# andrewmagis/snap-rnaseq

Measured on AMD Instinct MI355X. Metric: aligned reads/sec (100 bp SE, k=20 seed) at 1/2/4/8 GPUs + CPU baseline, higher is better.
Workload: dtype u8

## Files before the change

include/snapgpu.h:

```cpp
#ifndef SNAPGPU_H
#define SNAPGPU_H

#include <stddef.h>
#include <stdint.h>

#ifdef __cplusplus
extern "C" {
#endif

#define SNAPGPU_ABI_VERSION 2

enum {
    SNAPGPU_OK = 0,
    SNAPGPU_EINVAL = -1,
    SNAPGPU_EIO = -2,
    SNAPGPU_ENOMEM = -3,
    SNAPGPU_EDEVICE = -4,
    SNAPGPU_EFORMAT = -5,
    SNAPGPU_EUNSUPPORTED = -6
};

enum { SNAPGPU_NOT_FOUND = 0, SNAPGPU_SINGLE_HIT = 1, SNAPGPU_MULTIPLE_HITS = 2, SNAPGPU_UNKNOWN = 3 };
enum { SNAPGPU_FORWARD = 0, SNAPGPU_RC = 1 };

// ... 170 lines not shown
    uint32_t location;
    uint8_t  direction;
    uint8_t  score;
    uint16_t reserved;
} snapgpu_multi_hit_t;
int snapgpu_align_batch_ex(snapgpu_aligner_t *a, const snapgpu_reads_t *reads, const snapgpu_search_t *search,
                           uint32_t maxHitsToGet, snapgpu_result_t *out, int32_t *multiHitsFound,
                           snapgpu_multi_hit_t *multiHits);

typedef struct snapgpu_device_reads snapgpu_device_reads_t;
snapgpu_device_reads_t *snapgpu_reads_upload(snapgpu_aligner_t *a, const snapgpu_reads_t *reads);
void snapgpu_device_reads_free(snapgpu_device_reads_t *d);
int  snapgpu_align_resident(snapgpu_aligner_t *a, snapgpu_device_reads_t *d);
int  snapgpu_results_download(snapgpu_aligner_t *a, snapgpu_device_reads_t *d, snapgpu_result_t *out);
int  snapgpu_synchronize(snapgpu_aligner_t *a);

#define SNAPGPU_FASTQ_HOST_BATCH 1u
int snapgpu_fastq_upload(snapgpu_aligner_t *a, const char *text, uint64_t nBytes, const char *name,
                         int clipping, uint32_t flags,
                         snapgpu_device_reads_t **dOut, snapgpu_reads_t **readsOut);
int snapgpu_fastq_upload_file(snapgpu_aligner_t *a, const char *path, int clipping, uint32_t flags,
                              snapgpu_device_reads_t **dOut, snapgpu_reads_t **readsOut);
int snapgpu_fastq_upload_bgzf(snapgpu_aligner_t *a, const char *data, uint64_t nBytes, const char *name,
                              int clipping, uint32_t flags,
                              snapgpu_device_reads_t **dOut, snapgpu_reads_t **readsOut);
int snapgpu_fastq_upload_bgzf_file(snapgpu_aligner_t *a, const char *path, int clipping, uint32_t flags,
                                   snapgpu_device_reads_t **dOut, snapgpu_reads_t **readsOut);
int snapgpu_fastq_last_ms(snapgpu_aligner_t *a, double *uploadMs, double *kernelMs, double *downloadMs);
uint32_t snapgpu_fastq_tile_bytes(void);
int snapgpu_device_reads_peek(snapgpu_aligner_t *a, snapgpu_device_reads_t *d, uint64_t *n, uint64_t *bytes,
                              uint32_t *maxLen, uint64_t *extentHash, uint64_t *offsets, uint32_t *lengths,
                              char *bases, char *quals);
int snapgpu_device_reads_ids_download(snapgpu_aligner_t *a, snapgpu_device_reads_t *d, char *ids, uint64_t cap,
                                      uint64_t *used, uint64_t *idOffsets, uint32_t *idLengths,
                                      uint32_t *frontClipped, uint32_t *unclippedLength);

typedef struct snapgpu_timing {
    double mainKernelMs;
    double spillKernelMs;
    double fixupMs;
    uint64_t nSpilled;
    uint64_t nMapqFixed;
    double lookupKernelMs;
    uint64_t lookupSeeds;
    uint64_t lookupProbes;
    uint64_t lookupOverflowReads;
    uint64_t nLaunches;
    double wallMs;
    double mainKernelBusyMs;
    double lookupKernelBusyMs;
    uint64_t nByteReads;
    uint64_t nArenaOverflow;
    uint64_t nNulReads;
    uint64_t nUnwritten;
    uint64_t nForcedSettled;
    uint64_t nForcedLimitSpans;
    uint64_t nSimpleReads;
    uint64_t nSimpleBailed;
    uint64_t nSimpleWide;
} snapgpu_timing_t;
int snapgpu_last_timing(snapgpu_aligner_t *a, snapgpu_timing_t *t);

typedef struct snapgpu_aligner_stats {
    int64_t nHashTableLookups;
    int64_t nLocationsScored;
    int64_t nHitsIgnoredBecauseOfTooHighPopularity;
    int64_t nReadsIgnoredBecauseOfTooManyNs;
    int64_t nIndelsMerged;
    int64_t nReads;
} snapgpu_aligner_stats_t;
int snapgpu_aligner_get_stats(const snapgpu_aligner_t *a, snapgpu_aligner_stats_t *s);
int snapgpu_aligner_max_k(const snapgpu_aligner_t *a);
int snapgpu_aligner_set_overlap(snapgpu_aligner_t *a, int overlap);
int snapgpu_aligner_set_simple_pass(snapgpu_aligner_t *a, int on);
int snapgpu_aligner_debug_trip(snapgpu_aligner_t *a, uint32_t read_index);
typedef struct snapgpu_grids {
    uint32_t computeUnits, shortRows;
    uint32_t perCU128, grid128;
    uint32_t perCU256, grid256;
    uint32_t perCU512, grid512;
    uint32_t perCUSimple, gridSimple;
    uint32_t perCUCigar, gridCigar;
    uint32_t lds128, ldsUnit, ldsPerCU, reserved;
} snapgpu_grids_t;
int snapgpu_aligner_debug_grids(snapgpu_aligner_t *a, snapgpu_grids_t *g);
const char *snapgpu_source_sha256(void);
int snapgpu_phase_cycles(snapgpu_aligner_t *a, uint64_t *out, uint32_t len, int reset);
const char *snapgpu_aligner_name(const snapgpu_aligner_t *a);

int snapgpu_lv_batch(int device, int direction, uint32_t n,
                     const char *texts, const uint64_t *textOff, const uint32_t *textLen,
                     const char *patterns, const char *quals, const uint64_t *patOff,
                     const uint32_t *patLen, const int32_t *k,
                     int32_t *outScore, int32_t *outNetIndel, double *outProb);

#define SNAPGPU_LV_PASS_GROUPS 8
int snapgpu_lv_pass_batch(int device, int nw, uint32_t nPasses, const char *reads, const char *quals,
                          uint64_t readBytes, const uint64_t *readOff, const uint32_t *readLen,
                          const int32_t *seedLen, const int32_t *k, const char *genome, uint64_t genomeBytes,
                          const int64_t *cand, int32_t *outE1, int32_t *outE2, double *outP1, double *outP2,
                          int32_t *outNetIndel);

int snapgpu_lv_filter_batch(snapgpu_aligner_t *a, int quad, uint32_t nTasks, const char *reads, uint64_t readBytes,
                            const uint64_t *readOff, const uint32_t *readLen, const uint32_t *loc,
                            const int32_t *dir, const int32_t *s, const int32_t *k, const int32_t *act,
                            uint32_t *out);

#define SNAPGPU_CIGAR_MAX_OPS 64

int snapgpu_cigar_batch(snapgpu_aligner_t *a, const snapgpu_reads_t *reads, const uint32_t *locations,
                        const uint8_t *directions, int useM, int32_t *editDistance, uint32_t *nOps, uint32_t *ops);
int snapgpu_cigar_resident(snapgpu_aligner_t *a, snapgpu_device_reads_t *d, int useM);
int snapgpu_cigar_download(snapgpu_aligner_t *a, snapgpu_device_reads_t *d, int32_t *editDistance, uint32_t *nOps,
                           uint32_t *ops);
int snapgpu_cigar_last_ms(snapgpu_aligner_t *a, double *ms);

int snapgpu_sam_format(const snapgpu_index_t *idx, const snapgpu_reads_t *reads, const char *ids,
                       const uint64_t *idOffsets, const uint32_t *idLengths, const snapgpu_result_t *results,
                       const int32_t *editDistance, const uint32_t *nOps, const uint32_t *ops,
                       const char *readGroup, char *out, uint64_t cap, uint64_t *used);

int snapgpu_reads_clip(snapgpu_reads_t *reads, int clipping, uint32_t *frontClipped, uint32_t *unclippedLength);
int snapgpu_sam_format_clipped(const snapgpu_index_t *idx, const snapgpu_reads_t *reads, const char *ids,
                               const uint64_t *idOffsets, const uint32_t *idLengths, const snapgpu_result_t *results,
                               const int32_t *editDistance, const uint32_t *nOps, const uint32_t *ops,
                               const char *readGroup, const uint32_t *frontClipped, const uint32_t *unclippedLength,
                               char *out, uint64_t cap, uint64_t *used);

int snapgpu_sam_resident(snapgpu_aligner_t *a, snapgpu_device_reads_t *d, const snapgpu_reads_t *reads,
                         const char *ids, const uint64_t *idOffsets, const uint32_t *idLengths,
                         const char *readGroup);
int snapgpu_sam_download(snapgpu_aligner_t *a, snapgpu_device_reads_t *d, char *out, uint64_t cap, uint64_t *used);
int snapgpu_sam_format_gpu(snapgpu_aligner_t *a, const snapgpu_reads_t *reads, const char *ids,
                           const uint64_t *idOffsets, const uint32_t *idLengths, const snapgpu_result_t *results,
                           const int32_t *editDistance, const uint32_t *nOps, const uint32_t *ops,
                           const char *readGroup, const uint32_t *frontClipped, const uint32_t *unclippedLength,
                           char *out, uint64_t cap, uint64_t *used);
int snapgpu_sam_last_ms(snapgpu_aligner_t *a, double *kernelMs, double *downloadMs);
int snapgpu_sam_pass_ms(snapgpu_aligner_t *a, double *lengthMs, double *scanMs, double *writeMs);

int snapgpu_sam_resident_sorted(snapgpu_aligner_t *a, snapgpu_device_reads_t *d, const snapgpu_reads_t *reads,
                                const char *ids, const uint64_t *idOffsets, const uint32_t *idLengths,
                                const char *readGroup);
int snapgpu_sam_order_download(snapgpu_aligner_t *a, snapgpu_device_reads_t *d, uint32_t *order);
int snapgpu_sam_format_gpu_sorted(snapgpu_aligner_t *a, const snapgpu_reads_t *reads, const char *ids,
                                  const uint64_t *idOffsets, const uint32_t *idLengths, const snapgpu_result_t *results,
                                  const int32_t *editDistance, const uint32_t *nOps, const uint32_t *ops,
                                  const char *readGroup, const uint32_t *frontClipped, const uint32_t *unclippedLength,
                                  char *out, uint64_t cap, uint64_t *used, uint32_t *order);
int snapgpu_sam_sort_keys(const snapgpu_index_t *idx, uint64_t n, const snapgpu_result_t *results, uint32_t *keys);
int snapgpu_sam_sort_ms(snapgpu_aligner_t *a, double *sortMs);
int snapgpu_sam_line_lengths(const snapgpu_index_t *idx, const snapgpu_reads_t *reads, const char *ids,
                             const uint64_t *idOffsets, const uint32_t *idLengths, const snapgpu_result_t *results,
                             const int32_t *editDistance, const uint32_t *nOps, const uint32_t *ops,
                             const char *readGroup, const uint32_t *frontClipped, const uint32_t *unclippedLength,
                             uint32_t *lineLengths);

int snapgpu_sam_header(const snapgpu_index_t *idx, int sorted, const char *commandLine, const char *version,
                       const char *rgLine, char *out, uint64_t cap, uint64_t *used);

int snapgpu_bam_format(const snapgpu_index_t *idx, const snapgpu_reads_t *reads, const char *ids,
                       const uint64_t *idOffsets, const uint32_t *idLengths, const snapgpu_result_t *results,
                       const int32_t *editDistance, const uint32_t *nOps, const uint32_t *ops, const char *readGroup,
                       const uint32_t *frontClipped, const uint32_t *unclippedLength, int32_t nmCarryIn,
                       int32_t *nmCarryOut, char *out, uint64_t cap, uint64_t *used);
int snapgpu_bam_record_lengths(const snapgpu_index_t *idx, const snapgpu_reads_t *reads, const char *ids,
// ... 269 lines not shown
```

snap-rnaseq_amd/csrc/aligner.hip:

```cpp
#include <hip/hip_runtime.h>

#include <chrono>
#include <cmath>
#include <cstring>
#include <algorithm>
#include <atomic>
#include <mutex>
#include <string>
#include <thread>
#include <type_traits>
#include <vector>

#include "align_device.h"
#include "align_score.h"
#include "seed_lookup.h"
#include "simple_align.h"
#include "cigar.h"
#include "internal.h"
#include "resident_grid.h"
#include "large_copy.h"
#include "aligner_state.h"

using namespace sgk;
using snapgpu::uploadLarge;
// ... 2664 lines not shown
                            const int32_t *s, const int32_t *k, const int32_t *act, uint32_t *out) {
    if (!a || !a->dGPlanes) { snapgpu::setError("lv_filter_batch: no aligner"); return SNAPGPU_EINVAL; }
    if (nTasks == 0) return SNAPGPU_OK;
    const snapgpu_index_t *idx = a->idx;
    const int seedLen = (int)idx->seedLen;
    std::vector<LvfTask> tasks(nTasks);
    for (uint32_t i = 0; i < nTasks; i++) {
        const int64_t n = readLen[i];
        if (n < 1 || n > 128 || readOff[i] + (uint64_t)n > readBytes || (dir[i] != 0 && dir[i] != 1) || s[i] < 0 ||
            s[i] + seedLen > n || k[i] < 0 || k[i] > (quad ? LQ_K : FKM)) {
            snapgpu::setError("lv_filter_batch: read length 1..128, 0 <= s <= n - seedLen, 0 <= k <= 5 (pairs) / 7 (quads)");
            return SNAPGPU_EINVAL;
        }
        tasks[i] = LvfTask{readOff[i], loc[i], (int32_t)n, dir[i], s[i], k[i], act[i] != 0};
    }
    HIPCHK(hipSetDevice(a->device));
    LvfArgs A;
    A.gpl = a->dGPlanes; A.pieces = a->dPieces; A.nPieces = (int32_t)idx->genome->pieceOffsets.size();
    A.nBases = idx->genome->nBases; A.padding = idx->genome->chromosomePadding; A.seedLen = (uint32_t)seedLen;
    LvfTask *dT = nullptr; char *dR = nullptr; uint32_t *dO = nullptr;
    int rc = SNAPGPU_OK;
    if (hipMalloc(&dT, nTasks * sizeof(LvfTask)) != hipSuccess || hipMalloc(&dR, readBytes + 64) != hipSuccess ||
        hipMalloc(&dO, (size_t)nTasks * 4) != hipSuccess) {
        snapgpu::setError("lv_filter_batch: hipMalloc");
        rc = SNAPGPU_ENOMEM;
    }
    if (!rc) {
        hipMemcpy(dT, tasks.data(), nTasks * sizeof(LvfTask), hipMemcpyHostToDevice);
        hipMemcpy(dR, reads, readBytes, hipMemcpyHostToDevice);
        const uint32_t per = quad ? 16u : 32u;
        const dim3 grid((nTasks + per - 1) / per);
        if (quad) hipLaunchKernelGGL(lv_filter_kernel<true>, grid, dim3(64), 0, 0, A, dT, nTasks, dR, dO);
        else hipLaunchKernelGGL(lv_filter_kernel<false>, grid, dim3(64), 0, 0, A, dT, nTasks, dR, dO);
        if (hipGetLastError() != hipSuccess || hipDeviceSynchronize() != hipSuccess) {
            snapgpu::setError("lv_filter_kernel failed");
            rc = SNAPGPU_EDEVICE;
        } else hipMemcpy(out, dO, (size_t)nTasks * 4, hipMemcpyDeviceToHost);
    }
    hipFree(dT); hipFree(dR); hipFree(dO);
    return rc;
}

static CigarArgs cigar_args(snapgpu_aligner_t *a, snapgpu_device_reads_t *d, int useM) {
    CigarArgs C;
    memset(&C, 0, sizeof(C));
    const snapgpu_index_t *idx = a->idx;
    C.genome = a->dGenome; C.pieces = a->dPieces; C.nPieces = (int32_t)idx->genome->pieceOffsets.size();
    C.nBases = idx->genome->nBases; C.padding = idx->genome->chromosomePadding;
    C.bases = d->dBases; C.offsets = d->dOffsets; C.lengths = d->dLengths; C.nReads = (uint32_t)d->n;
    C.useM = useM ? 1 : 0;
    return C;
}

static int cigar_grid(snapgpu_aligner_t *a) {
    if (!a->cigarGrid) {
        hipDeviceProp_t prop;
        HIPCHK(hipGetDeviceProperties(&prop, a->device));
        a->perCUCigar = resident_blocks_per_cu((const void *)cigar_kernel, 64, prop, 8);
        a->cigarGrid = prop.multiProcessorCount * a->perCUCigar;
    }
    return SNAPGPU_OK;
}

int snapgpu_aligner_debug_grids(snapgpu_aligner_t *a, snapgpu_grids_t *g) {
    if (!a || !g) { snapgpu::setError("debug_grids: null"); return SNAPGPU_EINVAL; }
    HIPCHK(hipSetDevice(a->device));
    if (int rc = cigar_grid(a)) return rc;
    hipDeviceProp_t prop;
    HIPCHK(hipGetDeviceProperties(&prop, a->device));
    g->computeUnits = (uint32_t)prop.multiProcessorCount;
    g->shortRows = a->shortRows ? 1u : 0u;
    g->perCU128 = (uint32_t)a->perCU128; g->grid128 = (uint32_t)a->grid;
    g->perCU256 = (uint32_t)a->perCU256; g->grid256 = (uint32_t)a->grid256;
    g->perCU512 = (uint32_t)a->perCU512; g->grid512 = (uint32_t)a->grid512;
    g->perCUSimple = (uint32_t)a->perCUSimple; g->gridSimple = (uint32_t)a->gridSimple;
    g->perCUCigar = (uint32_t)a->perCUCigar; g->gridCigar = (uint32_t)a->cigarGrid;
    hipFuncAttributes fa;
    HIPCHK(a->shortRows ? hipFuncGetAttributes(&fa, (const void *)align_kernel<128, false, SHORT_ROWS>)
                        : hipFuncGetAttributes(&fa, (const void *)align_kernel<128, false>));
    g->lds128 = (uint32_t)fa.sharedSizeBytes;
    g->ldsUnit = (uint32_t)LDS_ALLOC_UNIT;
    g->ldsPerCU = (uint32_t)prop.maxSharedMemoryPerMultiProcessor;
    g->reserved = 0;
    return SNAPGPU_OK;
}

static int cigar_kernel_launch(snapgpu_aligner_t *a, const CigarArgs &C, uint64_t n) {
    if (int rc = cigar_grid(a)) return rc;
    int grid = a->cigarGrid;
    if ((uint64_t)grid > n) grid = (int)n;
    if (grid == 0) return SNAPGPU_OK;
    HIPCHK(hipEventRecord(a->cev[0], a->sideStream));
    hipLaunchKernelGGL(cigar_kernel, dim3(grid), dim3(64), 0, a->sideStream, C);
    HIPCHK(hipGetLastError());
    HIPCHK(hipEventRecord(a->cev[1], a->sideStream));
    return SNAPGPU_OK;
}

static int cigar_launch(snapgpu_aligner_t *a, snapgpu_device_reads_t *d, CigarArgs C) {
    if (d->maxLen > (uint32_t)CIG_MAXLEN) { snapgpu::setError("cigar: read longer than 512 bases"); return SNAPGPU_EINVAL; }
    if (d->n > 0xffffffffull) { snapgpu::setError("batch too large"); return SNAPGPU_EINVAL; }
    if (!d->dCigEd) {
        HIPCHK(hipMalloc(&d->dCigEd, (d->n + 1) * 4));
        HIPCHK(hipMalloc(&d->dCigN, (d->n + 1) * 4));
        HIPCHK(hipMalloc(&d->dCigOps, (d->n + 1) * CIG_MAX_OPS * 4));
    }
    C.outEd = d->dCigEd; C.outNOps = d->dCigN; C.outOps = d->dCigOps;
    return cigar_kernel_launch(a, C, d->n);
}

int snapgpu_cigar_resident(snapgpu_aligner_t *a, snapgpu_device_reads_t *d, int useM) {
    if (!a || !d) return SNAPGPU_EINVAL;
    HIPCHK(hipSetDevice(a->device));
    if (a->failed) { snapgpu::setError("aligner failed earlier (device timeout)"); return SNAPGPU_EDEVICE; }
    for (auto &L : a->lane) {
        HIPCHK(hipEventRecord(L.done, L.stream));
        HIPCHK(hipStreamWaitEvent(a->sideStream, L.done, 0));
    }
    CigarArgs C = cigar_args(a, d, useM);
    C.records = d->dOut;
    const int rc = cigar_launch(a, d, C);
    if (rc) return rc;
    HIPCHK(hipEventRecord(a->residentSideDone, a->sideStream));
    a->residentSidePending = true;
    return SNAPGPU_OK;
}

int snapgpu_cigar_download(snapgpu_aligner_t *a, snapgpu_device_reads_t *d, int32_t *editDistance, uint32_t *nOps,
                           uint32_t *ops) {
    if (!a || !d || !editDistance || !nOps || !ops || !d->dCigEd) return SNAPGPU_EINVAL;
    HIPCHK(hipSetDevice(a->device));
    HIPCHK(hipStreamSynchronize(a->sideStream));
    HIPCHK(hipMemcpy(editDistance, d->dCigEd, d->n * 4, hipMemcpyDeviceToHost));
    HIPCHK(hipMemcpy(nOps, d->dCigN, d->n * 4, hipMemcpyDeviceToHost));
    HIPCHK(hipMemcpy(ops, d->dCigOps, d->n * CIG_MAX_OPS * 4, hipMemcpyDeviceToHost));
    return SNAPGPU_OK;
}

int snapgpu_cigar_last_ms(snapgpu_aligner_t *a, double *ms) {
    if (!a || !ms) return SNAPGPU_EINVAL;
    HIPCHK(hipSetDevice(a->device));
    HIPCHK(hipEventSynchronize(a->cev[1]));
    float f = 0;
    HIPCHK(hipEventElapsedTime(&f, a->cev[0], a->cev[1]));
    *ms = f;
    return SNAPGPU_OK;
}

int snapgpu_cigar_batch(snapgpu_aligner_t *a, const snapgpu_reads_t *reads, const uint32_t *locations,
                        const uint8_t *directions, int useM, int32_t *editDistance, uint32_t *nOps, uint32_t *ops) {
    if (!a || !reads || !locations || !directions || !editDistance || !nOps || !ops) return SNAPGPU_EINVAL;
    const char *const base[2] = {reads->bases, reads->bases};
    return snapgpu_internal_cigar_view(a, base, nullptr, reads->offsets, reads->lengths, reads->n, locations, directions,
                                       useM, editDistance, nOps, ops);
}

static int cigarPinned(snapgpu_aligner_t *a, const char *const base[2], const uint8_t *mate, const uint64_t *offsets,
                       const uint32_t *lengths, uint64_t n, const uint32_t *locations, const uint8_t *directions,
                       int useM, const int32_t **outEd, const uint32_t **outNOps, const uint32_t **outOps) {
    if (a->failed) { snapgpu::setError("aligner failed earlier (device timeout)"); return SNAPGPU_EDEVICE; }
    *outEd = nullptr; *outNOps = nullptr; *outOps = nullptr;
    if (n == 0) return SNAPGPU_OK;
    if (n > 0xffffffffull) { snapgpu::setError("batch too large"); return SNAPGPU_EINVAL; }
    HIPCHK(hipSetDevice(a->device));
    uint64_t total = 0;
    uint32_t maxLen = 0;
// ... 223 lines not shown
```

snap-rnaseq_amd/csrc/seed_lookup.h:

```cpp
#pragma once
#include "align_device.h"
#include "bucket_table.h"
#include "order_long.h"

namespace sgk {

constexpr int LOOKUP_WAVES = 4;

__device__ __forceinline__ uint32_t win128(uint64_t lo, uint64_t hi, int p, int len) {
    uint64_t w;
    if (p == 0) w = lo;
    else if (p < 64) w = (lo >> p) | (hi << (64 - p));
    else w = hi >> (p - 64);
    return (uint32_t)w & (uint32_t)((1ull << len) - 1);
}
__device__ __forceinline__ uint64_t spread2(uint32_t x32) {
    uint64_t x = x32;
    x = (x | (x << 16)) & 0x0000FFFF0000FFFFull;
    x = (x | (x << 8)) & 0x00FF00FF00FF00FFull;
    x = (x | (x << 4)) & 0x0F0F0F0F0F0F0F0Full;
    x = (x | (x << 2)) & 0x3333333333333333ull;
    x = (x | (x << 1)) & 0x5555555555555555ull;
    return x;
}

__global__ __launch_bounds__(64 * LOOKUP_WAVES) void seed_lookup_kernel(KArgs A, SeedRec *out, unsigned long long *stats) {
    __shared__ uint32_t wrapT[32];
    if (threadIdx.x < 32) wrapT[threadIdx.x] = A.tab->wrap[threadIdx.x];
    __syncthreads();
    const int lane = lane_id();
    const uint32_t r = (blockIdx.x * LOOKUP_WAVES + threadIdx.x / 64) * 4 + (lane >> 4);
    const int k = lane & 15;
    const int sub = k & 7;
    const bool have = r < A.nReads;
    const uint32_t n = have ? A.lengths[r] : 0;
    const uint64_t off = have ? A.offsets[r] : 0;
    const int L = (int)A.seedLen;
    uint64_t chunk = 0;
    bool bad = false;
    {
        const uint64_t b0 = off + 16 * (uint64_t)sub;
        const uint32_t *src = (const uint32_t *)(A.bases + (b0 & ~3ull));
        const uint32_t sh = (uint32_t)(b0 & 3) * 8;
        uint32_t w[5];
#pragma unroll
        for (int i = 0; i < 5; i++) w[i] = have && k < 8 && n > 16u * sub ? src[i] : 0u;
        uint32_t p0 = 0, p1 = 0, iv = 0;
        const int lim = (int)n - 16 * sub;
#pragma unroll
        for (int i = 0; i < 4; i++) {
            const uint32_t d = __builtin_amdgcn_alignbit(w[i + 1], w[i], sh);
#pragma unroll
            for (int b = 0; b < 4; b++) {
                const uint32_t c = (d >> (8 * b)) & 0xffu;
                const uint32_t uc = (c >= 'a' && c <= 'z') ? c - 0x20u : c;
                const uint32_t o = uc - 0x40u;
                constexpr uint32_t kAcgt = (1u << 1) | (1u << 3) | (1u << 7) | (1u << 20);
                const bool acgt = o < 32u && ((kAcgt >> (o & 31u)) & 1u);
                const uint32_t x0 = (uc >> 1) & 1u, x1 = (uc >> 2) & 1u;
                const int bit = 4 * i + b;
                const bool inside = bit < lim;
                const bool inv = !inside || !acgt;
                bad |= k < 8 && inside && !acgt;
                p0 |= (inv ? 0u : x1) << bit;
                p1 |= (inv ? 0u : (x0 ^ x1)) << bit;
                iv |= (inv ? 1u : 0u) << bit;
            }
        }
        chunk = (uint64_t)p0 | ((uint64_t)p1 << 16) | ((uint64_t)iv << 32);
    }
    SeedRec rec = {0u, 0u, 0u, 0u};
    uint32_t weight = 0;
    uint32_t nSeed = 0, nProbe = 0, nOvfRead = 0;
    const int grp = lane & ~15;
    const uint64_t badMask = ballot(bad);
    const bool can = have && (int)n >= L;
    const bool lng = n > 128;
    const int firstRound = 128 / L;
    int my = -1;
    uint32_t w0 = 0, w1 = 0;
    if (badMask == 0) {
        if (can && !lng) {
            const uint32_t t = A.tab->seedSeq[n][k];
            my = t == 0xffu ? -1 : (int)t;
        } else if (can) my = k < firstRound ? k * L : -1;
        const int c0 = my > 0 ? my >> 4 : 0;
        const uint32_t a = (uint32_t)shfl_idx((int)(uint32_t)chunk, grp + c0);
        const uint32_t b = (uint32_t)shfl_idx((int)(uint32_t)chunk, grp + (c0 + 1 < 8 ? c0 + 1 : 7));
        const uint32_t c = (uint32_t)shfl_idx((int)(uint32_t)chunk, grp + (c0 + 2 < 8 ? c0 + 2 : 7));
        const uint64_t q0 = (uint64_t)(a & 0xffffu) | ((uint64_t)(b & 0xffffu) << 16) | ((uint64_t)(c & 0xffffu) << 32);
        const uint64_t q1 = (uint64_t)(a >> 16) | ((uint64_t)(b >> 16) << 16) | ((uint64_t)(c >> 16) << 32);
        const int sh = my > 0 ? my - 16 * c0 : 0;
        const uint32_t M = (uint32_t)((1ull << L) - 1);
        w0 = (uint32_t)(q0 >> sh) & M;
        w1 = (uint32_t)(q1 >> sh) & M;
    } else {
        uint64_t P0[2] = {0, 0}, P1[2] = {0, 0}, IV[2] = {0, 0};
#pragma unroll
        for (int j = 0; j < 8; j++) {
            const int src = grp + j;
            const uint32_t lo = (uint32_t)shfl_idx((int)(uint32_t)chunk, src);
            const uint32_t hi = (uint32_t)shfl_idx((int)(uint32_t)(chunk >> 32), src);
            const int wd = j >> 2, s = 16 * (j & 3);
            P0[wd] |= (uint64_t)(lo & 0xffff) << s;
            P1[wd] |= (uint64_t)(lo >> 16) << s;
            IV[wd] |= (uint64_t)(hi & 0xffff) << s;
        }
        const bool clean = ((badMask >> grp) & 0xffffull) == 0;
        if (can) {
            const int nPossible = (lng ? 128 : (int)n) - L + 1;
            uint64_t u0 = 0, u1 = 0;
            int p = 0, wrap = 0, idx = 0;
            if (clean && lng) my = k < firstRound ? k * L : -1;
            else if (clean) {
                const uint32_t t = A.tab->seedSeq[n][k];
                my = t == 0xffu ? -1 : (int)t;
            }
#pragma nounroll
            for (int guard = 0; !clean && guard < 4 * 128; guard++) {
                if (p >= nPossible) {
                    if (lng || ++wrap >= L) break;
                    p = (int)wrapT[wrap];
                }
#pragma clang loop vectorize(disable) interleave(disable) unroll(disable)
                while (p < nPossible && (((p < 64 ? u0 >> p : u1 >> (p - 64)) & 1ull) != 0)) p++;
                if (p >= nPossible) continue;
                if (p < 64) u0 |= 1ull << p; else u1 |= 1ull << (p - 64);
                if (win128(IV[0], IV[1], p, L)) continue;
                if (idx == k) { my = p; break; }
                idx++;
                p += L;
            }
            if (my >= 0) { w0 = win128(P0[0], P0[1], my, L); w1 = win128(P1[0], P1[1], my, L); }
        }
    }
    {
        const uint32_t M = (uint32_t)((1ull << L) - 1);
        const uint32_t r0 = __builtin_bitreverse32(w0) >> (32 - L), r1 = __builtin_bitreverse32(w1) >> (32 - L);
        const uint64_t f = (spread2(r1) << 1) | spread2(r0);
        const uint64_t rcv = (spread2(~w1 & M) << 1) | spread2(~w0 & M);
        const bool comp = (int64_t)f > (int64_t)rcv;
        const uint64_t canon = comp ? rcv : f;
        const uint32_t table = (uint32_t)(canon >> 32);
        const uint32_t key = (uint32_t)canon;
        uint32_t v1 = 0, v2 = 0, aux = 0, probes = 0;
        const bool found = bucket_lookup_quad(A, my >= 0, table, key, v1, v2, aux, probes);
        if (my >= 0 && found && lng) {
            const uint32_t c1 = aux & BK_CSAT, c2 = (aux >> 15) & BK_CSAT;
            auto side = [&](uint32_t v, uint32_t c) -> uint32_t {
                return v == UNUSED_SIDE ? 0u : v < A.nBases ? 1u : c >= BK_CSAT ? 0xffffu : c;
            };
            const uint32_t h = side(v1, c1) + (f != rcv ? side(v2, c2) : 0u);
            weight = h <= A.maxHits ? h : 0u;
        }
        if (my >= 0) {
            uint32_t cnt = 0;
            nSeed = 1;
            nProbe = probes;
            if (found) {
                const uint32_t c1 = aux & BK_CSAT, c2 = (aux >> 15) & BK_CSAT;
                const uint32_t vf = comp ? v2 : v1, vr = comp ? v1 : v2;
                const uint32_t nf = comp ? c2 : c1, nr = comp ? c1 : c2;
                uint32_t cf = 0, cr = 0;
                if (vf >= A.nBases && vf != UNUSED_SIDE) { cf = bucket_count(A, nf, vf); nOvfRead += nf >= BK_CSAT; }
                if (f != rcv && vr >= A.nBases && vr != UNUSED_SIDE) { cr = bucket_count(A, nr, vr); nOvfRead += nr >= BK_CSAT; }
                cnt = (cf < 0xffffu ? cf : 0xffffu) | ((cr < 0xffffu ? cr : 0xffffu) << 16);
            }
            rec.meta = 0x80000000u | (uint32_t)my | (found ? 0x100u : 0u) | (comp ? 0x200u : 0u) |
                       (f == rcv ? 0x400u : 0u) | ((probes < 0x7fffu ? probes : 0x7fffu) << 16);
            rec.v1 = v1;
            rec.v2 = v2;
            rec.cnt = cnt;
        }
    }
    if (have) out[(uint64_t)r * SEEDS_PER_READ + k] = rec;
    if (A.longCount) {
        const bool isLong = have && lng;
        const uint64_t ml = ballot(k == 0 && isLong);
        if (ml) {
            uint32_t w = weight;
#pragma unroll
            for (int s = 8; s >= 1; s >>= 1) w += (uint32_t)__shfl_xor((int)w, s, 64);
            uint32_t bl = 0;
            if (lane == 0) {
                bl = atomicAdd(A.deferCount, (uint32_t)__popcll(ml));
                atomicAdd(A.longCount, (uint32_t)__popcll(ml));
            }
            bl = (uint32_t)readlane((int)bl, 0);
            const uint32_t at = bl + (uint32_t)__popcll(ml & ((1ull << lane) - 1));
            if (k == 0 && isLong) {
                if (A.orderTmp) A.orderTmp[at] = r | (order_class(w) << ORDER_CLASS_SHIFT);
                else A.deferList[at] = r;
            }
        }
    }
    if (stats) {
        const uint32_t seeds = (uint32_t)__popcll(ballot(nSeed != 0));
        const uint32_t ovf = (uint32_t)__popcll(ballot(nOvfRead >= 1)) + (uint32_t)__popcll(ballot(nOvfRead >= 2));
        const uint32_t probes = sum_reduce32(nProbe);
        if (lane == 0) {
            unsigned long long *st = stats + 4 * ((blockIdx.x * LOOKUP_WAVES + threadIdx.x / 64) & 255);
            atomicAdd(st + 0, (unsigned long long)seeds);
            atomicAdd(st + 1, (unsigned long long)probes);
            atomicAdd(st + 2, (unsigned long long)ovf);
        }
    }
}

}
```

snap-rnaseq_amd/snapgpu/_ffi.py:

```python
import ctypes as C
import os

_HERE = os.path.dirname(os.path.abspath(__file__))
LIB_PATH = os.environ.get("SNAPGPU_LIB", os.path.join(_HERE, "libsnapgpu.so"))


class Result(C.Structure):
    _fields_ = [
        ("location", C.c_uint32),
        ("score", C.c_int32),
        ("mapq", C.c_int32),
        ("result", C.c_uint8),
        ("direction", C.c_uint8),
        ("flags", C.c_uint8),
        ("reserved", C.c_uint8),
        ("nLookups", C.c_uint32),
        ("nLocationsScored", C.c_uint32),
        ("popularSeedsSkipped", C.c_uint16),
        ("nHitsIgnored", C.c_uint16),
        ("nProbes", C.c_uint32),
        ("nHitWords", C.c_uint32),
        ("nOverflowLists", C.c_uint32),
        ("nElements", C.c_uint32),
        ("reserved2", C.c_uint32),
# ... 121 lines not shown
        ("mainKernelBusyMs", C.c_double),
        ("lookupKernelBusyMs", C.c_double),
        ("nByteReads", C.c_uint64),
        ("nArenaOverflow", C.c_uint64),
        ("nNulReads", C.c_uint64),
        ("nUnwritten", C.c_uint64),
        ("nForcedSettled", C.c_uint64),
        ("nForcedLimitSpans", C.c_uint64),
        ("nSimpleReads", C.c_uint64),
        ("nSimpleBailed", C.c_uint64),
        ("nSimpleWide", C.c_uint64),
    ]


class SingleOptions(C.Structure):
    _fields_ = [
        ("clipping", C.c_int32),
        ("confDiff", C.c_uint32),
        ("maxDist", C.c_uint32),
        ("minPercentAbovePhred", C.c_float),
        ("minPhred", C.c_uint32),
        ("phredOffset", C.c_uint32),
        ("useM", C.c_uint32),
        ("sortOutput", C.c_uint32),
        ("readGroup", C.c_char_p),
        ("commandLine", C.c_char_p),
        ("version", C.c_char_p),
        ("contaminationAligner", C.c_void_p),
        ("contaminants", C.c_void_p),
    ]


class RnaPairedOptions(C.Structure):
    _fields_ = [
        ("clipping", C.c_int32), ("confDiff", C.c_uint32), ("maxDist", C.c_uint32), ("minSpacing", C.c_uint32),
        ("maxSpacing", C.c_uint32), ("forceSpacing", C.c_uint32), ("minPercentAbovePhred", C.c_float),
        ("minPhred", C.c_uint32), ("phredOffset", C.c_uint32), ("useM", C.c_uint32), ("maxHitsToGet", C.c_uint32),
        ("ignoreMismatchedIDs", C.c_uint32), ("readGroup", C.c_char_p), ("commandLine", C.c_char_p),
        ("version", C.c_char_p), ("contaminationAligner", C.c_void_p), ("contaminants", C.c_void_p),
        ("sortOutput", C.c_uint32),
    ]


class RnaPairedStats(C.Structure):
    _fields_ = [(f, C.c_uint64) for f in ("totalPairs", "usefulPairs", "singleHits", "multiHits", "notFound",
                                          "transcriptomeRecords", "partialPairs", "partialMatches", "seedRuns")] + \
               [(f, C.c_double) for f in ("alignMs", "filterMs", "seedMs", "cigarMs", "writeMs", "wallMs", "prepMs",
                                           "countMs")] + [("subBatches", C.c_uint64)] + \
               [(f, C.c_double) for f in ("cigarGpuMs", "spliceMs")] + [("countedPairs", C.c_uint64)]


class SingleStats(C.Structure):
    _fields_ = [(f, C.c_uint64) for f in ("totalReads", "usefulReads", "singleHits", "multiHits", "notFound",
                                          "transcriptomeRecords")] + \
               [(f, C.c_double) for f in ("alignMs", "cigarMs", "filterMs", "writeMs", "wallMs", "prepMs", "formatMs", "ioMs")]


class SeedRuns(C.Structure):
    _fields_ = [("n", C.c_uint64), ("start", C.POINTER(C.c_uint64)), ("nForward", C.POINTER(C.c_uint32)),
                ("flags", C.POINTER(C.c_uint32)), ("runs", C.c_void_p), ("nRuns", C.c_uint64)]


class CharSeedsParams(C.Structure):
    _fields_ = [("maxHits", C.c_uint32), ("maxK", C.c_uint32), ("numSeeds", C.c_uint32), ("maxReadSize", C.c_uint32),
                ("explorePopularSeeds", C.c_uint32), ("reserved", C.c_uint32)]


class AlignerStats(C.Structure):
    _fields_ = [
        ("nHashTableLookups", C.c_int64),
        ("nLocationsScored", C.c_int64),
        ("nHitsIgnoredBecauseOfTooHighPopularity", C.c_int64),
        ("nReadsIgnoredBecauseOfTooManyNs", C.c_int64),
        ("nIndelsMerged", C.c_int64),
        ("nReads", C.c_int64),
    ]


assert C.sizeof(Result) == 64, C.sizeof(Result)

class Grids(C.Structure):
    _fields_ = [(f, C.c_uint32) for f in (
        "computeUnits", "shortRows", "perCU128", "grid128", "perCU256", "grid256", "perCU512", "grid512",
        "perCUSimple", "gridSimple", "perCUCigar", "gridCigar", "lds128", "ldsUnit", "ldsPerCU", "reserved")]


class BucketInfo(C.Structure):
    _fields_ = [("nSlots", C.c_uint64), ("nKeys", C.c_uint64), ("nBuckets", C.c_uint64),
                ("nOverflowBuckets", C.c_uint64), ("maxDisplacement", C.c_uint64), ("bytes", C.c_uint64),
                ("buildMs", C.c_double)]


INDEX_BUILD_PHASES = ("upload", "scan", "sort", "runs", "sizing", "placement", "write", "download")

_PROTOS = [
    ("snapgpu_abi_version", C.c_int, []),
    ("snapgpu_last_error", C.c_char_p, []),
    ("snapgpu_host_threads", C.c_int, []),
    ("snapgpu_aligner_params_default", None, [C.POINTER(AlignerParams)]),
    ("snapgpu_genome_from_fasta", C.c_void_p, [C.c_char_p, C.c_uint32]),
    ("snapgpu_genome_synthetic", C.c_void_p, [C.POINTER(SynthGenomeParams)]),
    ("snapgpu_genome_write_fasta", C.c_int, [C.c_void_p, C.c_char_p]),
    ("snapgpu_genome_free", None, [C.c_void_p]),
    ("snapgpu_genome_nbases", C.c_uint32, [C.c_void_p]),
    ("snapgpu_genome_bases", C.c_void_p, [C.c_void_p]),
    ("snapgpu_genome_npieces", C.c_int, [C.c_void_p]),
    ("snapgpu_genome_piece_offset", C.c_uint32, [C.c_void_p, C.c_int]),
    ("snapgpu_genome_piece_name", C.c_char_p, [C.c_void_p, C.c_int]),
    ("snapgpu_index_build", C.c_void_p, [C.c_void_p, C.c_int, C.c_int]),
    ("snapgpu_index_build_ex", C.c_void_p, [C.c_void_p, C.c_int, C.c_int, C.c_double]),
    ("snapgpu_index_build_gpu", C.c_void_p, [C.c_void_p, C.c_int, C.c_double, C.c_int]),
    ("snapgpu_index_build_gpu_stats", C.c_int, [C.POINTER(C.c_double), C.POINTER(C.c_uint64)]),
    ("snapgpu_index_load", C.c_void_p, [C.c_char_p]),
    ("snapgpu_index_share", C.c_int, [C.c_void_p, C.c_char_p]),
    ("snapgpu_index_attach", C.c_void_p, [C.c_char_p]),
    ("snapgpu_index_genome", C.c_void_p, [C.c_void_p]),
    ("snapgpu_index_save", C.c_int, [C.c_void_p, C.c_char_p]),
    ("snapgpu_index_free", None, [C.c_void_p]),
    ("snapgpu_index_get_info", C.c_int, [C.c_void_p, C.POINTER(IndexInfo)]),
    ("snapgpu_index_get_view", C.c_int, [C.c_void_p, C.POINTER(IndexView)]),
    ("snapgpu_index_lookup", C.c_int, [C.c_void_p, C.c_char_p, C.POINTER(C.c_uint32),
                                       C.POINTER(C.c_uint32), C.POINTER(C.c_uint32), C.c_uint32]),
    ("snapgpu_reads_synthetic", C.POINTER(Reads), [C.c_void_p, C.POINTER(SynthReadsParams)]),
    ("snapgpu_reads_synthetic_pairs", C.c_int, [C.c_void_p, C.POINTER(SynthReadsParams), C.c_uint32, C.c_uint32,
                                                C.POINTER(C.POINTER(Reads)), C.POINTER(C.POINTER(Reads))]),
    ("snapgpu_reads_from_fastq", C.POINTER(Reads), [C.c_char_p]),
    ("snapgpu_reads_from_fastq_buffer", C.POINTER(Reads), [C.c_void_p, C.c_uint64, C.c_char_p]),
    ("snapgpu_reads_from_arrays", C.POINTER(Reads), [C.c_uint64, C.c_char_p, C.c_char_p,
                                                     C.POINTER(C.c_uint64), C.POINTER(C.c_uint32)]),
    ("snapgpu_reads_write_fastq", C.c_int, [C.POINTER(Reads), C.c_char_p]),
    ("snapgpu_reads_free", None, [C.POINTER(Reads)]),
    ("snapgpu_device_count", C.c_int, []),
    ("snapgpu_device_cu_count", C.c_int, [C.c_int]),
    ("snapgpu_aligner_create", C.c_void_p, [C.c_int, C.c_void_p, C.POINTER(AlignerParams)]),
    ("snapgpu_aligner_free", None, [C.c_void_p]),
    ("snapgpu_align_batch", C.c_int, [C.c_void_p, C.POINTER(Reads), C.POINTER(Result)]),
    ("snapgpu_align_batch_submit", C.c_int, [C.c_void_p, C.POINTER(Reads), C.POINTER(Result)]),
    ("snapgpu_align_batch_wait", C.c_int, [C.c_void_p]),
    ("snapgpu_align_batch_ex", C.c_int, [C.c_void_p, C.POINTER(Reads), C.c_void_p, C.c_uint32, C.c_void_p, C.c_void_p,
                                         C.c_void_p]),
    ("snapgpu_reads_upload", C.c_void_p, [C.c_void_p, C.POINTER(Reads)]),
    ("snapgpu_device_reads_free", None, [C.c_void_p]),
    ("snapgpu_align_resident", C.c_int, [C.c_void_p, C.c_void_p]),
    ("snapgpu_results_download", C.c_int, [C.c_void_p, C.c_void_p, C.POINTER(Result)]),
    ("snapgpu_synchronize", C.c_int, [C.c_void_p]),
    ("snapgpu_fastq_upload", C.c_int, [C.c_void_p, C.c_void_p, C.c_uint64, C.c_char_p, C.c_int, C.c_uint32,
                                       C.POINTER(C.c_void_p), C.POINTER(C.POINTER(Reads))]),
    ("snapgpu_fastq_upload_file", C.c_int, [C.c_void_p, C.c_char_p, C.c_int, C.c_uint32,
                                            C.POINTER(C.c_void_p), C.POINTER(C.POINTER(Reads))]),
    ("snapgpu_fastq_upload_bgzf", C.c_int, [C.c_void_p, C.c_void_p, C.c_uint64, C.c_char_p, C.c_int, C.c_uint32,
                                            C.POINTER(C.c_void_p), C.POINTER(C.POINTER(Reads))]),
    ("snapgpu_fastq_upload_bgzf_file", C.c_int, [C.c_void_p, C.c_char_p, C.c_int, C.c_uint32,
                                                 C.POINTER(C.c_void_p), C.POINTER(C.POINTER(Reads))]),
    ("snapgpu_fastq_last_ms", C.c_int, [C.c_void_p, C.POINTER(C.c_double), C.POINTER(C.c_double),
                                        C.POINTER(C.c_double)]),
    ("snapgpu_fastq_tile_bytes", C.c_uint32, []),
    ("snapgpu_device_reads_peek", C.c_int, [C.c_void_p, C.c_void_p, C.POINTER(C.c_uint64), C.POINTER(C.c_uint64),
                                            C.POINTER(C.c_uint32), C.POINTER(C.c_uint64), C.c_void_p, C.c_void_p,
                                            C.c_void_p, C.c_void_p]),
    ("snapgpu_device_reads_ids_download", C.c_int, [C.c_void_p, C.c_void_p, C.c_void_p, C.c_uint64,
                                                    C.POINTER(C.c_uint64), C.c_void_p, C.c_void_p, C.c_void_p,
                                                    C.c_void_p]),
    ("snapgpu_last_timing", C.c_int, [C.c_void_p, C.POINTER(Timing)]),
    ("snapgpu_aligner_get_stats", C.c_int, [C.c_void_p, C.POINTER(AlignerStats)]),
    ("snapgpu_aligner_max_k", C.c_int, [C.c_void_p]),
    ("snapgpu_aligner_set_overlap", C.c_int, [C.c_void_p, C.c_int]),
    ("snapgpu_aligner_set_simple_pass", C.c_int, [C.c_void_p, C.c_int]),
# ... 200 lines not shown
```

Before: 68.38 million.

## Shrink seed lookup kernel to one wave per block and cut register pressure

Changes the seed lookup kernel to one 64-lane wave per block, so the block barrier becomes a wave sync. The packed 64-bit chunk is split into two 32-bit values. The clean-group window extraction now runs on a single shared path, and the dirty path only shuffles the invalid bits. Lane and read indices are recomputed before the epilogue to shorten live ranges. The aim is lower VGPR use and less divergence for higher occupancy, at the cost of four times as many small blocks. VGPR counts are also exposed through the debug grids struct.

Result: faster. 70.54 million (median of 6 runs) (+3.2%).

```diff
diff --git a/include/snapgpu.h b/include/snapgpu.h
--- a/include/snapgpu.h
+++ b/include/snapgpu.h
@@ -276,6 +276,7 @@
     uint32_t perCUSimple, gridSimple;
     uint32_t perCUCigar, gridCigar;
     uint32_t lds128, ldsUnit, ldsPerCU, reserved;
+    uint32_t vgprLookup, vgpr128;
 } snapgpu_grids_t;
 int snapgpu_aligner_debug_grids(snapgpu_aligner_t *a, snapgpu_grids_t *g);
 const char *snapgpu_source_sha256(void);
diff --git a/snap-rnaseq_amd/csrc/aligner.hip b/snap-rnaseq_amd/csrc/aligner.hip
--- a/snap-rnaseq_amd/csrc/aligner.hip
+++ b/snap-rnaseq_amd/csrc/aligner.hip
@@ -2770,6 +2770,9 @@
     g->ldsUnit = (uint32_t)LDS_ALLOC_UNIT;
     g->ldsPerCU = (uint32_t)prop.maxSharedMemoryPerMultiProcessor;
     g->reserved = 0;
+    g->vgpr128 = ((uint32_t)fa.numRegs + 7u) & ~7u;
+    HIPCHK(hipFuncGetAttributes(&fa, (const void *)seed_lookup_kernel));
+    g->vgprLookup = ((uint32_t)fa.numRegs + 7u) & ~7u;
     return SNAPGPU_OK;
 }
 
diff --git a/snap-rnaseq_amd/csrc/seed_lookup.h b/snap-rnaseq_amd/csrc/seed_lookup.h
--- a/snap-rnaseq_amd/csrc/seed_lookup.h
+++ b/snap-rnaseq_amd/csrc/seed_lookup.h
@@ -5,7 +5,7 @@
 
 namespace sgk {
 
-constexpr int LOOKUP_WAVES = 4;
+constexpr int LOOKUP_WAVES = 1;
 
 __device__ __forceinline__ uint32_t win128(uint64_t lo, uint64_t hi, int p, int len) {
     uint64_t w;
@@ -25,18 +25,20 @@
 }
 
 __global__ __launch_bounds__(64 * LOOKUP_WAVES) void seed_lookup_kernel(KArgs A, SeedRec *out, unsigned long long *stats) {
+    static_assert(LOOKUP_WAVES == 1, "wrapT is shared through wave_sync(): one wave per block");
     __shared__ uint32_t wrapT[32];
     if (threadIdx.x < 32) wrapT[threadIdx.x] = A.tab->wrap[threadIdx.x];
-    __syncthreads();
+    wave_sync();
     const int lane = lane_id();
-    const uint32_t r = (blockIdx.x * LOOKUP_WAVES + threadIdx.x / 64) * 4 + (lane >> 4);
+    const uint32_t r = blockIdx.x * 4 + (lane >> 4);
     const int k = lane & 15;
     const int sub = k & 7;
     const bool have = r < A.nReads;
     const uint32_t n = have ? A.lengths[r] : 0;
     const uint64_t off = have ? A.offsets[r] : 0;
     const int L = (int)A.seedLen;
-    uint64_t chunk = 0;
+    uint32_t chunk = 0;
+    uint32_t chunkIv = 0;
     bool bad = false;
     {
         const uint64_t b0 = off + 16 * (uint64_t)sub;
@@ -67,57 +69,40 @@
                 iv |= (inv ? 1u : 0u) << bit;
             }
         }
-        chunk = (uint64_t)p0 | ((uint64_t)p1 << 16) | ((uint64_t)iv << 32);
+        chunk = p0 | (p1 << 16);
+        chunkIv = iv;
+        asm volatile("" : "+v"(chunk), "+v"(chunkIv));
     }
     SeedRec rec = {0u, 0u, 0u, 0u};
     uint32_t weight = 0;
-    uint32_t nSeed = 0, nProbe = 0, nOvfRead = 0;
+    uint32_t nProbe = 0, nOvfRead = 0;
     const int grp = lane & ~15;
     const uint64_t badMask = ballot(bad);
     const bool can = have && (int)n >= L;
     const bool lng = n > 128;
     const int firstRound = 128 / L;
     int my = -1;
-    uint32_t w0 = 0, w1 = 0;
-    if (badMask == 0) {
-        if (can && !lng) {
+    const bool clean = ((badMask >> grp) & 0xffffull) == 0;
+    if (can && clean) {
+        if (lng) my = k < firstRound ? k * L : -1;
+        else {
             const uint32_t t = A.tab->seedSeq[n][k];
             my = t == 0xffu ? -1 : (int)t;
-        } else if (can) my = k < firstRound ? k * L : -1;
-        const int c0 = my > 0 ? my >> 4 : 0;
-        const uint32_t a = (uint32_t)shfl_idx((int)(uint32_t)chunk, grp + c0);
-        const uint32_t b = (uint32_t)shfl_idx((int)(uint32_t)chunk, grp + (c0 + 1 < 8 ? c0 + 1 : 7));
-        const uint32_t c = (uint32_t)shfl_idx((int)(uint32_t)chunk, grp + (c0 + 2 < 8 ? c0 + 2 : 7));
-        const uint64_t q0 = (uint64_t)(a & 0xffffu) | ((uint64_t)(b & 0xffffu) << 16) | ((uint64_t)(c & 0xffffu) << 32);
-        const uint64_t q1 = (uint64_t)(a >> 16) | ((uint64_t)(b >> 16) << 16) | ((uint64_t)(c >> 16) << 32);
-        const int sh = my > 0 ? my - 16 * c0 : 0;
-        const uint32_t M = (uint32_t)((1ull << L) - 1);
-        w0 = (uint32_t)(q0 >> sh) & M;
-        w1 = (uint32_t)(q1 >> sh) & M;
-    } else {
-        uint64_t P0[2] = {0, 0}, P1[2] = {0, 0}, IV[2] = {0, 0};
+        }
+    }
+    if (badMask != 0) {
+        uint64_t IV[2] = {0, 0};
 #pragma unroll
         for (int j = 0; j < 8; j++) {
-            const int src = grp + j;
-            const uint32_t lo = (uint32_t)shfl_idx((int)(uint32_t)chunk, src);
-            const uint32_t hi = (uint32_t)shfl_idx((int)(uint32_t)(chunk >> 32), src);
-            const int wd = j >> 2, s = 16 * (j & 3);
-            P0[wd] |= (uint64_t)(lo & 0xffff) << s;
-            P1[wd] |= (uint64_t)(lo >> 16) << s;
-            IV[wd] |= (uint64_t)(hi & 0xffff) << s;
-        }
-        const bool clean = ((badMask >> grp) & 0xffffull) == 0;
-        if (can) {
+            const uint32_t hi = (uint32_t)shfl_idx((int)chunkIv, grp + j);
+            IV[j >> 2] |= (uint64_t)(hi & 0xffff) << (16 * (j & 3));
+        }
+        if (can && !clean) {
             const int nPossible = (lng ? 128 : (int)n) - L + 1;
             uint64_t u0 = 0, u1 = 0;
             int p = 0, wrap = 0, idx = 0;
-            if (clean && lng) my = k < firstRound ? k * L : -1;
-            else if (clean) {
-                const uint32_t t = A.tab->seedSeq[n][k];
-                my = t == 0xffu ? -1 : (int)t;
-            }
 #pragma nounroll
-            for (int guard = 0; !clean && guard < 4 * 128; guard++) {
+            for (int guard = 0; guard < 4 * 128; guard++) {
                 if (p >= nPossible) {
                     if (lng || ++wrap >= L) break;
                     p = (int)wrapT[wrap];
@@ -131,8 +116,20 @@
                 idx++;
                 p += L;
             }
-            if (my >= 0) { w0 = win128(P0[0], P0[1], my, L); w1 = win128(P1[0], P1[1], my, L); }
-        }
+        }
+    }
+    uint32_t w0, w1;
+    {
+        const int c0 = my > 0 ? my >> 4 : 0;
+        const uint32_t a = (uint32_t)shfl_idx((int)chunk, grp + c0);
+        const uint32_t b = (uint32_t)shfl_idx((int)chunk, grp + (c0 + 1 < 8 ? c0 + 1 : 7));
+        const uint32_t c = (uint32_t)shfl_idx((int)chunk, grp + (c0 + 2 < 8 ? c0 + 2 : 7));
+        const uint64_t q0 = (uint64_t)(a & 0xffffu) | ((uint64_t)(b & 0xffffu) << 16) | ((uint64_t)(c & 0xffffu) << 32);
+        const uint64_t q1 = (uint64_t)(a >> 16) | ((uint64_t)(b >> 16) << 16) | ((uint64_t)(c >> 16) << 32);
+        const int sh = my > 0 ? my - 16 * c0 : 0;
+        const uint32_t M = (uint32_t)((1ull << L) - 1);
+        w0 = (uint32_t)(q0 >> sh) & M;
+        w1 = (uint32_t)(q1 >> sh) & M;
     }
     {
         const uint32_t M = (uint32_t)((1ull << L) - 1);
@@ -140,6 +137,7 @@
         const uint64_t f = (spread2(r1) << 1) | spread2(r0);
         const uint64_t rcv = (spread2(~w1 & M) << 1) | spread2(~w0 & M);
         const bool comp = (int64_t)f > (int64_t)rcv;
+        const bool pal = f == rcv;
         const uint64_t canon = comp ? rcv : f;
         const uint32_t table = (uint32_t)(canon >> 32);
         const uint32_t key = (uint32_t)canon;
@@ -150,12 +148,11 @@
             auto side = [&](uint32_t v, uint32_t c) -> uint32_t {
                 return v == UNUSED_SIDE ? 0u : v < A.nBases ? 1u : c >= BK_CSAT ? 0xffffu : c;
             };
-            const uint32_t h = side(v1, c1) + (f != rcv ? side(v2, c2) : 0u);
+            const uint32_t h = side(v1, c1) + (!pal ? side(v2, c2) : 0u);
             weight = h <= A.maxHits ? h : 0u;
         }
         if (my >= 0) {
             uint32_t cnt = 0;
-            nSeed = 1;
             nProbe = probes;
             if (found) {
                 const uint32_t c1 = aux & BK_CSAT, c2 = (aux >> 15) & BK_CSAT;
@@ -163,43 +160,45 @@
                 const uint32_t nf = comp ? c2 : c1, nr = comp ? c1 : c2;
                 uint32_t cf = 0, cr = 0;
                 if (vf >= A.nBases && vf != UNUSED_SIDE) { cf = bucket_count(A, nf, vf); nOvfRead += nf >= BK_CSAT; }
-                if (f != rcv && vr >= A.nBases && vr != UNUSED_SIDE) { cr = bucket_count(A, nr, vr); nOvfRead += nr >= BK_CSAT; }
+                if (!pal && vr >= A.nBases && vr != UNUSED_SIDE) { cr = bucket_count(A, nr, vr); nOvfRead += nr >= BK_CSAT; }
                 cnt = (cf < 0xffffu ? cf : 0xffffu) | ((cr < 0xffffu ? cr : 0xffffu) << 16);
             }
             rec.meta = 0x80000000u | (uint32_t)my | (found ? 0x100u : 0u) | (comp ? 0x200u : 0u) |
-                       (f == rcv ? 0x400u : 0u) | ((probes < 0x7fffu ? probes : 0x7fffu) << 16);
+                       (pal ? 0x400u : 0u) | ((probes < 0x7fffu ? probes : 0x7fffu) << 16);
             rec.v1 = v1;
             rec.v2 = v2;
             rec.cnt = cnt;
         }
     }
-    if (have) out[(uint64_t)r * SEEDS_PER_READ + k] = rec;
+    const int laneE = lane_id();
+    const uint32_t rE = blockIdx.x * 4 + (laneE >> 4);
+    if (rE < A.nReads) out[(uint64_t)rE * SEEDS_PER_READ + (laneE & 15)] = rec;
     if (A.longCount) {
         const bool isLong = have && lng;
-        const uint64_t ml = ballot(k == 0 && isLong);
+        const uint64_t ml = ballot((laneE & 15) == 0 && isLong);
         if (ml) {
             uint32_t w = weight;
 #pragma unroll
             for (int s = 8; s >= 1; s >>= 1) w += (uint32_t)__shfl_xor((int)w, s, 64);
             uint32_t bl = 0;
-            if (lane == 0) {
+            if (laneE == 0) {
                 bl = atomicAdd(A.deferCount, (uint32_t)__popcll(ml));
                 atomicAdd(A.longCount, (uint32_t)__popcll(ml));
             }
             bl = (uint32_t)readlane((int)bl, 0);
-            const uint32_t at = bl + (uint32_t)__popcll(ml & ((1ull << lane) - 1));
-            if (k == 0 && isLong) {
-                if (A.orderTmp) A.orderTmp[at] = r | (order_class(w) << ORDER_CLASS_SHIFT);
-                else A.deferList[at] = r;
+            const uint32_t at = bl + (uint32_t)__popcll(ml & ((1ull << laneE) - 1));
+            if ((laneE & 15) == 0 && isLong) {
+                if (A.orderTmp) A.orderTmp[at] = rE | (order_class(w) << ORDER_CLASS_SHIFT);
+                else A.deferList[at] = rE;
             }
         }
     }
     if (stats) {
-        const uint32_t seeds = (uint32_t)__popcll(ballot(nSeed != 0));
+        const uint32_t seeds = (uint32_t)__popcll(ballot(my >= 0));
         const uint32_t ovf = (uint32_t)__popcll(ballot(nOvfRead >= 1)) + (uint32_t)__popcll(ballot(nOvfRead >= 2));
         const uint32_t probes = sum_reduce32(nProbe);
-        if (lane == 0) {
-            unsigned long long *st = stats + 4 * ((blockIdx.x * LOOKUP_WAVES + threadIdx.x / 64) & 255);
+        if (laneE == 0) {
+            unsigned long long *st = stats + 4 * (blockIdx.x & 255);
             atomicAdd(st + 0, (unsigned long long)seeds);
             atomicAdd(st + 1, (unsigned long long)probes);
             atomicAdd(st + 2, (unsigned long long)ovf);
diff --git a/snap-rnaseq_amd/snapgpu/_ffi.py b/snap-rnaseq_amd/snapgpu/_ffi.py
--- a/snap-rnaseq_amd/snapgpu/_ffi.py
+++ b/snap-rnaseq_amd/snapgpu/_ffi.py
@@ -227,7 +227,8 @@
 class Grids(C.Structure):
     _fields_ = [(f, C.c_uint32) for f in (
         "computeUnits", "shortRows", "perCU128", "grid128", "perCU256", "grid256", "perCU512", "grid512",
-        "perCUSimple", "gridSimple", "perCUCigar", "gridCigar", "lds128", "ldsUnit", "ldsPerCU", "reserved")]
+        "perCUSimple", "gridSimple", "perCUCigar", "gridCigar", "lds128", "ldsUnit", "ldsPerCU", "reserved",
+        "vgprLookup", "vgpr128")]
 
 
 class BucketInfo(C.Structure):
```
